# espnet/espnet

Hardware: AMD Instinct MI355X
Metric: audio-seconds/sec (RTF^-1), Conformer-ASR, 10 s utterances (higher is better)
Workload: dtype bf16; 1 GPU; BASELINE.json configs[1]: Conformer-small (12x256d, 4 heads), HIP STFT/log-mel + HIP encoder + greedy CTC (G1) + hypotheses collated to the host, 32 x 10 s utterances per GPU per step, V=5000; batch_per_gpu=32, global_batch=32, parallelism=utterance-dp1

## Files before the change

### espnet_amd/asr/encoder/conformer_encoder.py

```python
import ctypes as C
import math
import os
import threading
import weakref
from typing import List, Optional, Tuple

import torch

from espnet_amd import lib as L
from espnet_amd.nets_utils import (SUBSAMPLING_CONVS, SUBSAMPLING_MIN_FRAMES, conv2d_subsampled_lengths,
                                   conv_out_size)
from espnet_amd.packing import PackedModule

_POS_PROJ_LOCK = threading.Lock()
_ENC_CALL_LOCK = threading.Lock()
_TLS = threading.local()

LN_EPS = 1e-12


class LayerNorm(torch.nn.LayerNorm):
    def __init__(self, nout):
        super().__init__(nout, eps=LN_EPS)


class _Conv2dSubsampling(torch.nn.Module):

# ... 410 lines not shown
    def _pack_current(self, pk) -> bool:
        stamp = getattr(pk, "ctc_stamp", None)
        return stamp is None or self.fused_ctc is None or stamp == self._ctc_version(self.fused_ctc)

    def _pack_subsampling(self, w, t, A, F):
        e, d = self.embed, self._output_size
        layer = getattr(self, "input_layer", "conv2d")
        w.subsample = {"conv2d": 4, "conv2d6": 6, "conv2d8": 8}[layer]
        w.legacy_relpos = int(getattr(self, "legacy_relpos", False))
        k2 = e.conv[2].weight.size(-1)
        t["conv2_w"] = A(e.conv[2].weight.permute(0, 2, 3, 1).reshape(d, k2 * k2 * d))
        t["conv2_b"] = F(e.conv[2].bias)
        if layer == "conv2d" and d in (256, 512) and self.em_dtype == L.EM_BF16:
            t["conv1_wf"] = A(pack_conv1_frags(e.conv[0].weight, e.conv[0].bias))
            t["conv2_wf"] = A(pack_conv2_frags(e.conv[2].weight.permute(0, 2, 3, 1).reshape(d, 9 * d)))
        if layer == "conv2d8":
            t["conv3_w"] = A(e.conv[4].weight.permute(0, 2, 3, 1).reshape(d, 9 * d))
            t["conv3_b"] = F(e.conv[4].bias)

    def _pos_projected(self, T: int, device, pk, pos: torch.Tensor) -> torch.Tensor:
        cache = self.__dict__.setdefault("_pos_proj_cache", {})
        lock = _POS_PROJ_LOCK
        key = (T, str(device), pk.serial)
        cur = torch.cuda.current_stream()
        with lock:
            ent = cache.get(key)
            if ent is not None:
                out, ev, sid, _ = ent
                if sid != cur.cuda_stream:
                    cur.wait_event(ev)
# ... 151 lines not shown
```

### espnet_amd/csrc/api.hip

```cpp
#include <stdlib.h>

#include <atomic>
#include <mutex>

#include "em_common.h"
#include "switches.h"

namespace {
EmSwitches read_switches() {
  auto on = [](const char* n) { return getenv(n) != nullptr; };
  auto num = [](const char* n, int dflt) { const char* e = getenv(n); return e ? atoi(e) : dflt; };
  EmSwitches s = {};
  s.attn2_stamps = on("EM_ATTN2_STAMPS"); s.block_stamps = on("EM_BLOCK_STAMPS"); s.ffn_stamps = on("EM_FFN_STAMPS");
  s.sub2_stamps = on("EM_SUB2_STAMPS");
  s.block_no_helpers = on("ESPNET_AMD_BLOCK_NO_HELPERS");
  s.sa_split = num("ESPNET_AMD_SA_SPLIT", 0); s.sa_group = num("ESPNET_AMD_SA_GROUP", 0);
  s.no_sa_tree = on("ESPNET_AMD_NO_SA_TREE"); s.sa_tree_min_rows = num("ESPNET_AMD_SA_TREE_MIN_ROWS", 200);
  s.no_attn2_large = on("ESPNET_AMD_NO_ATTN2_LARGE"); s.no_ffn_rows = on("ESPNET_AMD_NO_FFN_ROWS");
  s.no_rows_ctc = on("ESPNET_AMD_NO_ROWS_CTC"); s.frontend_v1 = on("ESPNET_AMD_FRONTEND_V1");
  s.gemm_stages = num("ESPNET_AMD_GEMM_STAGES", 0); s.gemm_bm = num("ESPNET_AMD_GEMM_BM", 0); s.no_mid_gemm = on("ESPNET_AMD_NO_MID_GEMM");
  s.mid_tile = num("ESPNET_AMD_MID_TILE", 0); s.lng_rt = num("ESPNET_AMD_LNG_RT", 0); s.lng_wide = num("ESPNET_AMD_LNG_WIDE", 256);
  s.no_src_lnq = on("ESPNET_AMD_NO_SRC_LNQ"); s.no_tail_fusion = on("ESPNET_AMD_NO_TAIL_FUSION");
  s.stream_no_fused = on("ESPNET_AMD_STREAM_NO_FUSED"); s.stream_mha_v1 = on("ESPNET_AMD_STREAM_MHA_V1");
  s.stream_no_ctx_fold = on("ESPNET_AMD_STREAM_NO_CTX_FOLD"); s.stream_no_ln_gemm = on("ESPNET_AMD_STREAM_NO_LN_GEMM");
  s.stream_fused_min = num("ESPNET_AMD_STREAM_FUSED_MIN", 1); s.no_sub12 = on("ESPNET_AMD_NO_SUB12");
  s.stream_ffn_split = num("ESPNET_AMD_STREAM_FFN_SPLIT", 0); s.stream_split_att = on("ESPNET_AMD_STREAM_SPLIT_ATT");
  s.stream_tf_merge = num("ESPNET_AMD_STREAM_TF_MERGE", -1);
  s.dec_ffn_split = num("ESPNET_AMD_DEC_FFN_SPLIT", 0); s.dec_ffn_rows = num("ESPNET_AMD_DEC_FFN_ROWS", 0); s.no_rows_qkv = on("ESPNET_AMD_NO_ROWS_QKV"); s.ffn_rows_min_fill = num("ESPNET_AMD_FFN_ROWS_MIN_FILL", 0);
  return s;
}
std::atomic<const EmSwitches*> g_sw{nullptr};
std::mutex g_sw_mu;
}

const EmSwitches& em_sw() {
  const EmSwitches* p = g_sw.load(std::memory_order_acquire);
  if (!p) {
    std::lock_guard<std::mutex> lk(g_sw_mu);
    p = g_sw.load(std::memory_order_acquire);
    if (!p) {
// ... 50 lines not shown
```

### espnet_amd/csrc/ebranchformer.hip

```cpp
#include <math.h>
#include <stdlib.h>

#include "em_common.h"
#include "switches.h"
#include "subsample.h"

namespace {

constexpr float LN_EPS = 1e-12f;

inline size_t align_up(size_t v) { return (v + 255) & ~(size_t)255; }

struct Ws {
  size_t c1, c2, c3, x, xn, xn2, big, gn, gated, cat, tmp, ctx, pall, mw, qh, kh, vt, total;
  int Tpad;
};
inline Ws layout(int dtype, const EmEBranchformerWeights* w, int B, int T_f) {
  const size_t es = dtype == EM_BF16 ? 2 : 4;
  em_sub::Geo g;
  em_sub::geo(w->subsample, T_f, w->n_mels, &g);
  const size_t M = (size_t)B * g.T_out, d = w->d;
  size_t mb[3];
  em_sub::map_bytes(g, B, w->d, es, mb);
  size_t wide = w->ff > 3 * w->d ? w->ff : 3 * w->d;
// ... 155 lines not shown
  void* c1 = ws + s.c1;
  void* c2 = ws + s.c2;
  void* c3 = ws + s.c3;
  float* x = (float*)(ws + s.x);
  void* xn = ws + s.xn;
  void* xn2 = ws + s.xn2;
  void* big = ws + s.big;
  void* gn = ws + s.gn;
  void* gated = ws + s.gated;
  unsigned char* cat = ws + s.cat;
  void* tmp = ws + s.tmp;
  void* ctx = ws + s.ctx;
  void* pall = ws + s.pall;
  const size_t es = dtype == EM_BF16 ? 2 : 4;

  EM_TRY(em_sub::run(dtype, w, g, feats, mvn_partial, flens, B, c1, c2, c3, x, stream, w->conv1_wf, w->conv2_wf));
  EM_TRY(gemm(dtype, EM_EPI_STORE, pos_emb, w->wpos_all, pall, nullptr, w->legacy_relpos ? T : 2 * T - 1, L * d, d, d, L * d, 1.f,
              stream));
  const EmEBranchformerLayer* ly = w->layers;
  const bool ffn = w->use_ffn != 0;
  const bool no_attn2 = em_sw().no_attn2_large;
  const bool attn2 = dtype == EM_BF16 && !w->legacy_relpos && !no_attn2 && !(flags & EM_ENC_NO_FUSED) && d == 64 * h &&
                     (size_t)B * d * s.Tpad * 4 < ((size_t)1 << 32) - 64;
  void* qh = ws + s.qh;
  void* vt = ws + s.vt;
  if (attn2 && hipMemsetAsync(qh, 0, (s.vt - s.qh) + (size_t)B * d * s.Tpad * es, (hipStream_t)stream) != hipSuccess)
    return EM_ERR_LAUNCH;
  bool ffn_rows = ffn && dtype == EM_BF16 && d == 512 && ff % 128 == 0 && ff >= 256 && !(flags & EM_ENC_NO_FUSED) &&
                  !em_sw().no_ffn_rows && em_rows_fill_ok(M, flags);
  for (int l = 0; ffn_rows && l < L; ++l) ffn_rows = ly[l].ffm_w1p && ly[l].ffm_w2p && ly[l].ff_w1p && ly[l].ff_w2p;
  const EmEBranchformerLayer* ln_in = nullptr;
// ... 105 lines not shown
```

### espnet_amd/csrc/em_common.h

```cpp
#pragma once
#include <hip/hip_runtime.h>
#include <stdint.h>

#include <mutex>

#include "../../include/espnet_amd.h"

typedef __bf16 bf16;
typedef __attribute__((ext_vector_type(8))) __bf16 bf16x8;
typedef __attribute__((ext_vector_type(4))) __bf16 bf16x4;
typedef __attribute__((ext_vector_type(2))) __bf16 bf16x2;
typedef __attribute__((ext_vector_type(4))) float f32x4;
typedef __attribute__((ext_vector_type(2))) float f32x2;

#define EM_WAVE 64

template <typename T>
struct Mma;

template <>
struct Mma<bf16> {
  static constexpr int K = 32;
  static constexpr int EPL = 8;
  typedef bf16x8 frag;
// ... 124 lines not shown
  int dev = 0;
  if (hipGetDevice(&dev) != hipSuccess || dev < 0 || dev >= 64) return EM_ERR_LAUNCH;
  if ((int)bytes > __atomic_load_n(&cap->bytes[dev], __ATOMIC_ACQUIRE)) {
    std::lock_guard<std::mutex> lk(em_lds_cap_mu);
    if ((int)bytes > __atomic_load_n(&cap->bytes[dev], __ATOMIC_RELAXED)) {
      if (hipFuncSetAttribute(fn, hipFuncAttributeMaxDynamicSharedMemorySize, (int)bytes) != hipSuccess) return EM_ERR_LAUNCH;
      __atomic_store_n(&cap->bytes[dev], (int)bytes, __ATOMIC_RELEASE);
    }
  }
  return EM_OK;
}

bool em_prof_begin(void* stream);
void em_prof_end(void* stream, double flops, int tag);

bool em_rows_fill_ok(long M, int flags);

int em_dec_pack_memory_frag_bf16(const void* kv, int B, int T, int Tpad, int d, int heads, void* kf, void* vf, void* stream);
int em_dec_src_attention_lnq_memfrag_bf16(const float* x, const float* g, const float* be, float eps, const void* wq_frag,
                                          const float* bq, const void* kf, const void* vf, const int32_t* klens, int B, int W, int d,
                                          int heads, int T, int Tpad, void* ctx, void* stream);

int em_gemm_mid_frag(int epilogue, int frag, const EmGemmArgs* p, void* stream);

int em_dec_self_attention_tree_bf16(const void* qkv, void* kc, void* vc, const int* anc, const int* anc_odd, int n, int d,
                                    int heads, int Lmax, int pos, const int* pos_dev, int W, void* ctx, void* stream);

struct NgSearchArgs {
  int32_t n, W, V, Lmax, S, NC;
  float w_ctc, w_ngram;
  const int32_t* step;
// ... 10 lines not shown
```

### espnet_amd/csrc/encoder.hip

```cpp
#include <math.h>
#include <stdlib.h>

#include "em_common.h"
#include "switches.h"
#include "subsample.h"

namespace {

constexpr float LN_EPS = 1e-12f;

inline size_t align_up(size_t v) { return (v + 255) & ~(size_t)255; }

struct Ws {
  size_t c1, c2, c3, x, xn, big, g, g2, ctx, pall, qh, kh, vt, ppk, total;
  int Tpad;
};
inline int fused_tpad(int T) { return (T + 255) / 256 * 256; }
inline Ws layout(int dtype, const EmConformerWeights* w, int B, int T_f) {
  const size_t es = dtype == EM_BF16 ? 2 : 4;
  em_sub::Geo g;
  em_sub::geo(w->subsample, T_f, w->n_mels, &g);
  const size_t M = (size_t)B * g.T_out, d = w->d;
  size_t mb[3];
  em_sub::map_bytes(g, B, w->d, es, mb);
// ... 20 lines not shown
  return s;
}

inline int gemm(int dtype, int epi, const void* A, const void* W, void* C, const float* bias, int M,
                int N, int K, int lda, int ldc, float scale, void* stream) {
  EmGemmArgs a = {};
  a.A = A; a.W = W; a.C = C; a.bias = bias;
  a.M = M; a.N = N; a.K = K; a.lda = lda; a.ldc = ldc; a.scale = scale;
  a.T1 = a.F1 = a.T2 = a.F2 = a.d = 0;
  return em_gemm(dtype, epi, EM_A_PLAIN, &a, stream);
}


}

bool em_rows_fill_ok(long M, int flags) {
  static int n_cu_of[64] = {};
  int dev = 0;
  if (hipGetDevice(&dev) != hipSuccess || dev < 0 || dev >= 64) dev = 0;
  if (n_cu_of[dev] == 0) {
    hipDeviceProp_t prop;
    n_cu_of[dev] = (hipGetDeviceProperties(&prop, dev) == hipSuccess && prop.multiProcessorCount > 0) ? prop.multiProcessorCount : 256;
  }
  const int n_cu = n_cu_of[dev];
  int n = (flags >> 8) & 15;
  n = n < 1 ? 1 : n;
  const int forced = em_sw().ffn_rows_min_fill;
  const long fill = forced > 0 ? forced : 72 / n;
  const long wgs = (M + 63) / 64, rounds = (wgs + n_cu - 1) / n_cu;
  return M > 0 && 100 * wgs >= fill * rounds * n_cu;
}

namespace {

struct RowsPlan {
  bool ffn, pre_pw2, glu, ctc;
};
inline RowsPlan rows_plan(int dtype, const EmConformerWeights* w, int flags, long M) {
  RowsPlan r = {false, false, false, false};
  const bool no_ffn_rows = em_sw().no_ffn_rows;
  const int d = w->d, ff = w->ff, L = w->num_blocks;
  const EmConformerLayer* ly = w->layers;
  if (!(dtype == EM_BF16 && d == 512 && ff % 128 == 0 && ff >= 256 && !(flags & EM_ENC_NO_FUSED) && !no_ffn_rows && ly && L > 0 &&
        M > 0))
// ... 68 lines not shown
  if (!em_sub::geo(w->subsample, T_f, w->n_mels, &g)) return EM_ERR_UNSUPPORTED;
  const int T = g.T_out, M = B * T;
  unsigned char* ws = (unsigned char*)workspace;
  void* c1 = ws + s.c1;
  void* c2 = ws + s.c2;
  void* c3 = ws + s.c3;
  float* x = (float*)(ws + s.x);
  void* xn = ws + s.xn;
  void* big = ws + s.big;
  void* gl = ws + s.g;
  void* g2 = ws + s.g2;
  void* ctx = ws + s.ctx;
  void* pall = ws + s.pall;
  const size_t es = dtype == EM_BF16 ? 2 : 4;

  EM_TRY(em_sub::run(dtype, w, g, feats, mvn_partial, flens, B, c1, c2, c3, x, stream, w->conv1_wf, w->conv2_wf));
  const EmConformerLayer* ly = w->layers;
  if (flags & EM_ENC_POS_PROJECTED)
    pall = const_cast<void*>(pos_emb);
  else
    EM_TRY(gemm(dtype, EM_EPI_STORE, pos_emb, w->wpos_all, pall, nullptr, w->legacy_relpos ? T : 2 * T - 1, L * d, d, d,
                L * d, 1.f, stream));
  const int plan = encode_plan(dtype, w, flags);
  const bool fused = (plan & EM_ENC_PLAN_FUSED) != 0;
  if (fused) {
    void* qh = ws + s.qh;
    void* kh = ws + s.kh;
    void* vt = ws + s.vt;
    if (32 * em_cdiv(T, 32) < s.Tpad &&
        hipMemsetAsync(vt, 0, (size_t)B * d * s.Tpad * es, (hipStream_t)stream) != hipSuccess)
      return EM_ERR_LAUNCH;
// ... 176 lines not shown
```

### espnet_amd/csrc/subsample.h

```cpp
#pragma once
#include "switches.h"
#include <math.h>
#include <stdlib.h>

#include "em_common.h"

namespace em_sub {

struct Geo {
  int n;
  int T[4], F[4];
  int k[3], s[3];
  int T_out, F_out;
};

inline int mode_of(int subsample) { return subsample == 0 ? 4 : subsample; }

inline int min_frames(int subsample) {
  switch (mode_of(subsample)) {
    case 6: return 11;
    case 8: return 15;
    default: return 7;
  }
}
// ... 12 lines not shown
    g->F[i + 1] = (g->F[i] - g->k[i]) / g->s[i] + 1;
    if (g->T[i] < g->k[i] || g->F[i] < g->k[i]) return false;
  }
  g->T_out = g->T[convs];
  g->F_out = g->F[convs];
  return g->T_out >= 1 && g->F_out >= 1;
}

inline void map_bytes(const Geo& g, int B, int d, size_t es, size_t out[3]) {
  for (int i = 0; i < 3; ++i) out[i] = i <= g.n ? (size_t)B * g.T[i + 1] * g.F[i + 1] * d * es : 0;
}

template <typename W>
inline int run(int dtype, const W* w, const Geo& g, const float* feats, const float* mvn_partial,
               const int32_t* flens, int B, void* c1, void* c2, void* c3, float* x, void* stream,
               const void* conv1_wf = nullptr, const void* conv2_wf = nullptr) {
  const int d = w->d;
  int rc = EM_ERR_UNSUPPORTED;
  const bool no_fused = em_sw().no_sub12;
  const bool try_fused = dtype == EM_BF16 && conv1_wf && conv2_wf && mode_of(w->subsample) == 4 && !no_fused;
  if (try_fused)
    rc = em_conv2d_sub12_bf16(feats, mvn_partial, flens, B, g.T[0], g.F[0], conv1_wf, conv2_wf, w->conv2_b, d, c2, stream);
  if (rc != EM_OK && rc != EM_ERR_UNSUPPORTED) return rc;
  const bool fused = rc == EM_OK;
  if (!fused) {
    rc = em_conv2d_sub1(dtype, feats, mvn_partial, flens, B, g.T[0], g.F[0], w->conv1_w, w->conv1_b, d, c1, stream);
    if (rc != EM_OK) return rc;
  }
  const void* in = fused ? c2 : c1;
  void* outs[2] = {c2, c3};
  const void* ws[2] = {w->conv2_w, w->conv3_w};
  const float* bs[2] = {w->conv2_b, w->conv3_b};
  for (int i = fused ? 1 : 0; i < g.n; ++i) {
    EmGemmArgs a = {};
    a.A = in; a.W = ws[i]; a.C = outs[i]; a.bias = bs[i];
    a.M = B * g.T[i + 2] * g.F[i + 2]; a.N = d; a.K = g.k[i + 1] * g.k[i + 1] * d; a.lda = 0; a.ldc = d; a.scale = 1.f;
    a.T1 = g.T[i + 1]; a.F1 = g.F[i + 1]; a.T2 = g.T[i + 2]; a.F2 = g.F[i + 2]; a.d = d;
    a.conv_k = g.k[i + 1]; a.conv_s = g.s[i + 1];
    if (!a.W || !a.C) return EM_ERR_BAD_ARG;
    rc = em_gemm(dtype, EM_EPI_RELU, EM_A_CONV2, &a, stream);
    if (rc != EM_OK) return rc;
    in = outs[i];
  }
  EmGemmArgs e = {};
  e.A = in; e.W = w->embed_w; e.C = x; e.bias = w->embed_b;
  e.M = B * g.T_out; e.N = d; e.K = g.F_out * d; e.lda = g.F_out * d; e.ldc = d; e.scale = sqrtf((float)d);
  return em_gemm(dtype, EM_EPI_SCALE_F32, EM_A_PLAIN, &e, stream);
}

}
```

### espnet_amd/csrc/switches.h

```cpp
#pragma once

struct EmSwitches {
  bool attn2_stamps, block_stamps, ffn_stamps, sub2_stamps;
  bool block_no_helpers;
  int sa_split, sa_group;
  bool no_sa_tree;
  int sa_tree_min_rows;
  bool no_rows_qkv;
  bool no_attn2_large, no_ffn_rows, no_rows_ctc;
  bool frontend_v1;
  int gemm_stages, gemm_bm;
  bool no_mid_gemm;
  int mid_tile, lng_rt, lng_wide;
  bool no_src_lnq, no_tail_fusion;
  bool stream_no_fused, stream_mha_v1, stream_no_ctx_fold, stream_no_ln_gemm;
  int stream_fused_min;
  bool stream_split_att;
  int stream_ffn_split;
  int stream_tf_merge;
  bool no_sub12;
  int ffn_rows_min_fill;
  int dec_ffn_rows;
  int dec_ffn_split;
};

const EmSwitches& em_sw();
```

### espnet_amd/csrc/transformer.hip

```cpp
#include <math.h>
#include <stdlib.h>

#include "em_common.h"
#include "switches.h"
#include "subsample.h"

namespace {

constexpr float LN_EPS = 1e-12f;

inline size_t align_up(size_t v) { return (v + 255) & ~(size_t)255; }

struct Ws {
  size_t c1, c2, c3, x, xn, big, ctx, qh, kh, vt, total;
  int Tpad;
};
inline Ws layout(int dtype, const EmTransformerWeights* w, int B, int T_f) {
  const size_t es = dtype == EM_BF16 ? 2 : 4;
  em_sub::Geo g;
  em_sub::geo(w->subsample, T_f, w->n_mels, &g);
  const size_t M = (size_t)B * g.T_out, d = w->d;
  size_t mb[3];
  em_sub::map_bytes(g, B, w->d, es, mb);
  const size_t wide = (size_t)w->ff > 3 * d ? (size_t)w->ff : 3 * d;
// ... 64 lines not shown
  em_sub::Geo g;
  if (!em_sub::geo(w->subsample, T_f, w->n_mels, &g)) return EM_ERR_UNSUPPORTED;
  const int T = g.T_out, M = B * T;
  const size_t es = dtype == EM_BF16 ? 2 : 4;
  unsigned char* ws = (unsigned char*)workspace;
  float* x = (float*)(ws + s.x);
  void* xn = ws + s.xn;
  void* big = ws + s.big;
  void* ctx = ws + s.ctx;
  void* qh = ws + s.qh;
  void* kh = ws + s.kh;
  void* vt = ws + s.vt;
  hipStream_t hs = (hipStream_t)stream;

  EM_TRY(em_sub::run(dtype, w, g, feats, mvn_partial, flens, B, ws + s.c1, ws + s.c2, ws + s.c3, x, stream, w->conv1_wf,
                     w->conv2_wf));
  {
    const long n4 = (long)M * d / 4;
    hipLaunchKernelGGL(abs_pe_add_kernel, dim3((unsigned)((n4 + 255) / 256)), dim3(256), 0, hs, x, (const float*)pos_emb, T,
                       d / 4, n4);
    EM_CHECK_LAUNCH();
  }
  const EmTransformerLayer* ly = w->layers;
  if (L == 0)
    return em_layernorm(dtype, x, w->after_norm_g, w->after_norm_b, M, d, LN_EPS, enc_act, enc_out, stream);

  const bool heads_path = dtype == EM_BF16 && !em_sw().no_attn2_large && (size_t)B * d * s.Tpad * 4 < ((size_t)1 << 32) - 64;
  bool ffn_rows = dtype == EM_BF16 && d == 512 && ff % 128 == 0 && ff >= 256 && !(flags & EM_ENC_NO_FUSED) &&
                  !em_sw().no_ffn_rows && em_rows_fill_ok(M, flags);
  for (int l = 0; ffn_rows && l < L; ++l) ffn_rows = ly[l].ff_w1p && ly[l].ff_w2p;

// ... 43 lines not shown
```

### espnet_amd/lib.py

```python
import ctypes as C
import os
from pathlib import Path

_LIB_PATH = Path(__file__).resolve().parent / "lib" / "libespnet_amd.so"

EM_OK = 0
EM_LNF_RELU_FRAG, EM_LNF_STORE, EM_LNF_STORE_F32 = 0, 1, 2
EM_ERR_UNSUPPORTED, EM_ERR_BAD_ARG, EM_ERR_TOO_SHORT, EM_ERR_LAUNCH, EM_ERR_WORKSPACE, EM_ERR_IO = -1, -2, -3, -4, -5, -6
EM_F32, EM_BF16 = 0, 1
(EM_EPI_STORE, EM_EPI_SWISH, EM_EPI_RELU, EM_EPI_RESID_F32, EM_EPI_SCALE_F32, EM_EPI_GLU,
 EM_EPI_STORE_F32, _EM_EPI_UNUSED_7, _EM_EPI_UNUSED_8, EM_EPI_ARGMAX_PART, EM_EPI_GELU, EM_EPI_QK_HEADS,
 EM_EPI_VT_HEADS) = range(13)
EM_A_PLAIN, EM_A_CONV2 = 0, 1

EM_DW_SWISH, EM_DW_LINEAR, EM_DW_GATE, EM_DW_SELFRES = range(4)
EM_ENC_ISOLATE_UTTS = 1
EM_ENC_NO_FUSED = 2
EM_ENC_POS_PROJECTED = 4
EM_ENC_FOLD_C = 8
EM_ENC_SPLIT_ATT = 16
EM_ENC_POS_PACKED = 32


def EM_ENC_IN_FLIGHT(n):
# ... 64 lines not shown
               [(n, C.c_void_p) for n in ("pre_in", "pre_w", "pre_b", "pre_g", "pre_be")] + [("main", C.c_int32)] + \
               [(n, C.c_void_p) for n in ("post_w", "post_b", "post_ids")] + [("post_chunks", C.c_int32), ("post_vocab", C.c_int32)] + \
               [(n, C.c_void_p) for n in ("post_q", "post_k", "post_vt")] + [("post_T", C.c_int32), ("post_Tpad", C.c_int32)] + \
               [("act", C.c_int32)]


class EmConformerWeights(C.Structure):
    _fields_ = [("d", C.c_int32), ("heads", C.c_int32), ("ff", C.c_int32),
                ("num_blocks", C.c_int32), ("kernel", C.c_int32), ("n_mels", C.c_int32),
                ("conv1_w", C.c_void_p), ("conv1_b", C.c_void_p), ("conv2_w", C.c_void_p),
                ("conv2_b", C.c_void_p), ("embed_w", C.c_void_p), ("embed_b", C.c_void_p),
                ("wpos_all", C.c_void_p), ("after_norm_g", C.c_void_p),
                ("after_norm_b", C.c_void_p), ("layers", C.POINTER(EmConformerLayer)),
                ("subsample", C.c_int32), ("conv3_w", C.c_void_p), ("conv3_b", C.c_void_p),
                ("legacy_relpos", C.c_int32), ("ctc_w", C.c_void_p), ("ctc_b", C.c_void_p),
                ("ctc_ids", C.c_void_p), ("ctc_units", C.c_int32), ("conv1_wf", C.c_void_p), ("conv2_wf", C.c_void_p)]


_EBF_LAYER_PTRS = ["norm_ff_mac_g", "norm_ff_mac_b", "norm_mha_g", "norm_mha_b", "norm_mlp_g", "norm_mlp_b",
                   "norm_ff_g", "norm_ff_b", "norm_final_g", "norm_final_b", "ffm_w1", "ffm_w2", "ff_w1", "ff_w2",
                   "ffm_b1", "ffm_b2", "ff_b1", "ff_b2", "wqkv", "bqkv", "pos_u", "pos_v", "wout", "bout",
                   "proj1_w", "proj1_b", "csgu_norm_g", "csgu_norm_b", "csgu_conv_w", "csgu_conv_b", "proj2_w",
                   "proj2_b", "merge_conv_w", "merge_conv_b", "merge_w", "merge_b", "pool_w", "pool_b", "wproj_w",
                   "wproj_b", "ffm_w1p", "ffm_w2p", "ff_w1p", "ff_w2p", "wqkvp"]
EM_MERGE_CONCAT, EM_MERGE_LEARNED_AVE = 0, 1


class EmEBranchformerLayer(C.Structure):
    _fields_ = [(n, C.c_void_p) for n in _EBF_LAYER_PTRS]


class EmEBranchformerWeights(C.Structure):
    _fields_ = [(n, C.c_int32) for n in ("d", "heads", "ff", "cg", "num_blocks", "cg_kernel", "merge_kernel",
                                         "n_mels")] + \
               [(n, C.c_void_p) for n in ("conv1_w", "conv1_b", "conv2_w", "conv2_b", "embed_w", "embed_b",
                                          "wpos_all", "after_norm_g", "after_norm_b")] + \
               [("layers", C.POINTER(EmEBranchformerLayer)), ("use_ffn", C.c_int32), ("merge_conv", C.c_int32),
                ("subsample", C.c_int32), ("conv3_w", C.c_void_p), ("conv3_b", C.c_void_p),
                ("legacy_relpos", C.c_int32), ("merge_method", C.c_int32), ("conv1_wf", C.c_void_p),
                ("conv2_wf", C.c_void_p)]


_TRF_LAYER_PTRS = ["norm1_g", "norm1_b", "norm2_g", "norm2_b", "wqkv", "bqkv", "wout", "bout", "ff_w1", "ff_w2", "ff_b1",
                   "ff_b2", "ff_w1p", "ff_w2p", "cb_wqkvp", "cb_woutp", "cb_ff_w1p", "cb_ff_w2p", "fp_t"]


class EmTransformerLayer(C.Structure):
    _fields_ = [(n, C.c_void_p) for n in _TRF_LAYER_PTRS]


class EmTransformerWeights(C.Structure):
    _fields_ = [(n, C.c_int32) for n in ("d", "heads", "ff", "num_blocks", "n_mels", "subsample")] + \
               [(n, C.c_void_p) for n in ("conv1_w", "conv1_b", "conv2_w", "conv2_b", "conv3_w", "conv3_b", "embed_w",
                                          "embed_b", "after_norm_g", "after_norm_b")] + \
               [("layers", C.POINTER(EmTransformerLayer)), ("conv1_wf", C.c_void_p), ("conv2_wf", C.c_void_p)]


class EmWavInfo(C.Structure):
    _fields_ = [("frames", C.c_int64), ("data_offset", C.c_int64), ("rate", C.c_int32), ("channels", C.c_int32),
                ("bits", C.c_int32), ("format", C.c_int32), ("status", C.c_int32)]


_DEC_LAYER_PTRS = ["norm1_g", "norm1_b", "norm2_g", "norm2_b", "norm3_g", "norm3_b", "self_wqkv",
                   "self_bqkv", "self_wout", "self_bout", "src_wq", "src_bq", "src_wkv", "src_bkv",
                   "src_wout", "src_bout", "w1", "b1", "w2", "b2", "w1_frag", "w2_frag", "self_wqkv_frag",
                   "self_wout_frag", "src_wout_frag", "src_wq_frag"]


def pack_frag16(w, pad_rows=16):
    import torch
# ... 79 lines not shown
class EmSearchBuffers(C.Structure):
    _fields_ = [(n, C.c_void_p) for n in SEARCH_BUFFERS]


_i32, _f32, _vp, _sz = C.c_int32, C.c_float, C.c_void_p, C.c_size_t
_SIGNATURES = {
    "em_version": (C.c_int, []),
    "em_error_string": (C.c_char_p, [C.c_int]),
    "em_frontend_logmel_f32": (C.c_int, [_vp, _i32, _i32, _i32, _vp, _vp, _vp, _i32, _i32, _vp, _vp,
                                         _i32, _vp, _vp]),
    "em_utt_mvn_partial_f32": (C.c_int, [_vp, _vp, _i32, _i32, _i32, _vp, _vp]),
    "em_utt_mvn_apply_f32": (C.c_int, [_vp, _vp, _vp, _i32, _i32, _i32, _vp]),
    "em_global_mvn_f32": (C.c_int, [_vp, _vp, _vp, _vp, _i32, _i32, _i32, _vp]),
    "em_conv2d_sub1": (C.c_int, [C.c_int, _vp, _vp, _vp, _i32, _i32, _i32, _vp, _vp, _i32, _vp, _vp]),
    "em_conv2d_sub12_bf16": (C.c_int, [_vp, _vp, _vp, _i32, _i32, _i32, _vp, _vp, _vp, _i32, _vp, _vp]),
    "em_gemm": (C.c_int, [C.c_int, C.c_int, C.c_int, C.POINTER(EmGemmArgs), _vp]),
    "em_layernorm": (C.c_int, [C.c_int, _vp, _vp, _vp, _i32, _i32, _f32, _vp, _vp, _vp]),
    "em_layernorm2": (C.c_int, [C.c_int, _vp, _vp, _vp, _vp, _vp, _i32, _i32, _f32, _vp, _vp, _vp]),
    "em_layernorm_inplace_f32": (C.c_int, [_vp, _vp, _vp, _i32, _i32, _f32, _vp]),
    "em_relpos_attention": (C.c_int, [C.c_int, _vp, _vp, _i32, _vp, _vp, _vp, _i32, _i32, _i32,
                                      _i32, _vp, _vp]),
    "em_legacy_relpos_attention": (C.c_int, [C.c_int, _vp, _vp, _i32, _vp, _vp, _vp, _i32, _i32, _i32,
                                      _i32, _vp, _vp]),
    "em_dwconv_bn_swish": (C.c_int, [C.c_int, _vp, _vp, _vp, _vp, _i32, _i32, _i32, _i32, _vp, _vp]),
    "em_argmax_rows_f32": (C.c_int, [_vp, _i32, _i32, _vp, _vp]),
    "em_argmax_partials": (C.c_int, [_vp, _i32, _i32, _vp, _vp]),
    "em_log_softmax_rows_f32": (C.c_int, [_vp, _i32, _i32, _vp]),
    "em_ctc_collapse": (C.c_int, [_vp, _vp, _i32, _i32, _i32, _i32, _vp, _vp, _vp]),
    "em_conformer_workspace_bytes": (_sz, [C.c_int, C.POINTER(EmConformerWeights), _i32, _i32]),
    "em_ebranchformer_workspace_bytes": (_sz, [C.c_int, C.POINTER(EmEBranchformerWeights), _i32, _i32]),
# ... 156 lines not shown
```

### espnet_amd/packing.py

```python
import itertools
import threading

import torch

from espnet_amd import lib as L

_BUILD_LOCK = threading.RLock()
_SERIALS = itertools.count(1)


class Pack:

    def __init__(self, device: torch.device, dtype, act: torch.dtype, pe_len):
        self.device, self.dtype, self.act, self.pe_len = device, dtype, act, pe_len
        self.serial = next(_SERIALS)
        self.w = self.layers = None
        self.keep = []
        self._held = set()
        self._frozen = False

    def __setattr__(self, name, value):
        if self.__dict__.get("_frozen"):
            raise AttributeError(f"a pack does not change once built ({name})")
        object.__setattr__(self, name, value)
# ... 64 lines not shown
```

### include/espnet_amd.h

```cpp
#ifndef ESPNET_AMD_H_
#define ESPNET_AMD_H_

#include <stddef.h>
#include <stdint.h>

#ifdef __cplusplus
extern "C" {
#endif

#define EM_OK 0
#define EM_ERR_UNSUPPORTED (-1)
#define EM_ERR_BAD_ARG (-2)
#define EM_ERR_TOO_SHORT (-3)
#define EM_ERR_LAUNCH (-4)
#define EM_ERR_WORKSPACE (-5)
#define EM_ERR_IO (-6)

#define EM_F32 0
#define EM_BF16 1

#define EM_EPI_STORE 0
#define EM_EPI_SWISH 1
#define EM_EPI_RELU 2
#define EM_EPI_RESID_F32 3
// ... 33 lines not shown
                           int32_t n_mels, float* partial, void* stream);

int em_utt_mvn_apply_f32(float* feats, const float* partial, const int32_t* flens, int32_t B,
                         int32_t T_f, int32_t n_mels, void* stream);

int em_global_mvn_f32(float* feats, const int32_t* flens, const float* mean, const float* stdv,
                      int32_t B, int32_t T_f, int32_t n_mels, void* stream);

int em_conv2d_sub12_bf16(const float* feats, const float* mvn_partial, const int32_t* flens, int32_t B, int32_t T_f,
                         int32_t n_mels, const void* conv1_wf, const void* conv2_wf, const float* conv2_b, int32_t d,
                         void* c2, void* stream);

int em_conv2d_sub1(int dtype, const float* feats, const float* partial, const int32_t* flens,
                   int32_t B, int32_t T_f, int32_t n_mels, const float* w1, const float* b1,
                   int32_t d, void* out, void* stream);

int em_gemm(int dtype, int epilogue, int a_mode, const EmGemmArgs* args, void* stream);

int em_layernorm(int dtype, const float* x, const float* g, const float* b, int32_t M, int32_t d,
                 float eps, void* out, float* out_f32, void* stream);
int em_layernorm2(int dtype, float* x, const float* g1, const float* b1, const float* g2,
                  const float* b2, int32_t M, int32_t d, float eps, void* out, float* out_f32,
                  void* stream);

int em_layernorm_inplace_f32(float* x, const float* g, const float* b, int32_t M, int32_t d,
                             float eps, void* stream);

int em_ln_gemm(int dtype, int epilogue, const float* x, const float* ln_g, const float* ln_b, float eps,
               const void* W, const float* bias, void* C, int32_t M, int32_t N, int32_t K, int32_t ldc,
               void* stream);
// ... 70 lines not shown
  const void* embed_w;
  const float* embed_b;
  const void* wpos_all;
  const float *after_norm_g, *after_norm_b;
  const EmConformerLayer* layers;
  int32_t subsample;
  const void* conv3_w;
  const float* conv3_b;
  int32_t legacy_relpos;
  const void* ctc_w;
  const float* ctc_b;
  int32_t* ctc_ids;
  int32_t ctc_units;
  const void* conv1_wf;
  const void* conv2_wf;
} EmConformerWeights;

#define EM_ENC_ISOLATE_UTTS 1
#define EM_ENC_NO_FUSED 2
#define EM_ENC_FOLD_C 8
#define EM_ENC_SPLIT_ATT 16
#define EM_ENC_POS_PACKED 32
#define EM_ENC_POS_PROJECTED 4
#define EM_ENC_IN_FLIGHT(n) (((n) & 15) << 8)

#define EM_ENC_PLAN_FUSED 1
#define EM_ENC_PLAN_CTC_IDS 2
int em_conformer_encode_plan(int dtype, const EmConformerWeights* w, int32_t flags);
int em_conformer_encode_plan_for(int dtype, const EmConformerWeights* w, int32_t flags, int32_t B, int32_t T_f);

// ... 108 lines not shown

typedef struct EmTransformerWeights {
  int32_t d, heads, ff, num_blocks, n_mels;
  int32_t subsample;
  const float *conv1_w, *conv1_b;
  const void* conv2_w;
  const float* conv2_b;
  const void* conv3_w;
  const float* conv3_b;
  const void* embed_w;
  const float* embed_b;
  const float *after_norm_g, *after_norm_b;
  const EmTransformerLayer* layers;
  const void* conv1_wf;
  const void* conv2_wf;
} EmTransformerWeights;

size_t em_transformer_workspace_bytes(int dtype, const EmTransformerWeights* w, int32_t B, int32_t T_f);
int em_transformer_encode(int dtype, const EmTransformerWeights* w, const float* feats, const float* mvn_partial,
                          const int32_t* flens, const int32_t* olens, int32_t B, int32_t T_f, const void* pos_emb,
                          void* workspace, size_t workspace_bytes, float* enc_out, void* enc_act, int32_t flags,
                          void* stream);

typedef struct EmEBranchformerLayer {
  const float *norm_ff_mac_g, *norm_ff_mac_b, *norm_mha_g, *norm_mha_b, *norm_mlp_g, *norm_mlp_b;
  const float *norm_ff_g, *norm_ff_b, *norm_final_g, *norm_final_b;
  const void *ffm_w1, *ffm_w2, *ff_w1, *ff_w2;
  const float *ffm_b1, *ffm_b2, *ff_b1, *ff_b2;
  const void* wqkv;
  const float* bqkv;
// ... 25 lines not shown
  const float* conv2_b;
  const void* embed_w;
  const float* embed_b;
  const void* wpos_all;
  const float *after_norm_g, *after_norm_b;
  const EmEBranchformerLayer* layers;
  int32_t use_ffn;
  int32_t merge_conv;
  int32_t subsample;
  const void* conv3_w;
  const float* conv3_b;
  int32_t legacy_relpos;
  int32_t merge_method;
  const void* conv1_wf;
  const void* conv2_wf;
} EmEBranchformerWeights;

int em_branch_learned_ave(int dtype, const void* cat, const int32_t* lens, int32_t B, int32_t T, int32_t d,
                          const float* pool_w, const float* pool_b, const float* wproj_w,
                          const float* wproj_b, float* mw_ws, void* out, void* stream);

size_t em_ebranchformer_workspace_bytes(int dtype, const EmEBranchformerWeights* w, int32_t B, int32_t T_f);
int em_ebranchformer_encode(int dtype, const EmEBranchformerWeights* w, const float* feats,
                            const float* mvn_partial, const int32_t* flens, const int32_t* olens,
                            int32_t B, int32_t T_f, const void* pos_emb, void* workspace,
                            size_t workspace_bytes, float* enc_out, void* enc_act, int32_t flags,
                            void* stream);

int em_ctc_greedy(int dtype, const void* enc_act, const void* w_ctc, const float* b_ctc, int32_t B,
                  int32_t T, int32_t d, int32_t V, const int32_t* olens, int32_t blank,
// ... 300 lines not shown
```

Before: 354,700 audio-s/s.

## Add row-tiled MFMA kernel for subsampling embed projection with pre-packed weights

Adds a dedicated bf16 kernel for the Conv2dSubsampling output linear (embed) projection. It streams activation tiles into LDS with global_load_lds through a 4-stage ring and keeps pre-packed weight fragments in a register ring, fusing bias and sqrt(d) scaling into the store. Weights are repacked on the host at pack time into the fragment order. The kernel is used when the CU fill heuristic allows it, otherwise the generic GEMM runs. It aims to cut the generic GEMM's cost on this large-K, small-N shape, at the price of more code and a new packed-weight buffer.

```diff
diff --git a/espnet_amd/asr/encoder/conformer_encoder.py b/espnet_amd/asr/encoder/conformer_encoder.py
--- a/espnet_amd/asr/encoder/conformer_encoder.py
+++ b/espnet_amd/asr/encoder/conformer_encoder.py
@@ -10,7 +10,7 @@
 from espnet_amd import lib as L
 from espnet_amd.nets_utils import (SUBSAMPLING_CONVS, SUBSAMPLING_MIN_FRAMES, conv2d_subsampled_lengths,
                                    conv_out_size)
-from espnet_amd.packing import PackedModule
+from espnet_amd.packing import PackedModule, pack_embed_rows
 
 _POS_PROJ_LOCK = threading.Lock()
 _ENC_CALL_LOCK = threading.Lock()
@@ -451,6 +451,9 @@
         if layer == "conv2d" and d in (256, 512) and self.em_dtype == L.EM_BF16:
             t["conv1_wf"] = A(pack_conv1_frags(e.conv[0].weight, e.conv[0].bias))
             t["conv2_wf"] = A(pack_conv2_frags(e.conv[2].weight.permute(0, 2, 3, 1).reshape(d, 9 * d)))
+        F_out = e.out.in_features // d
+        if d in (256, 512) and self.em_dtype == L.EM_BF16 and (F_out * d) % 256 == 0:
+            t["embed_wf"] = A(pack_embed_rows(e.out.weight.reshape(d, d, F_out).permute(0, 2, 1).reshape(d, F_out * d)))
         if layer == "conv2d8":
             t["conv3_w"] = A(e.conv[4].weight.permute(0, 2, 3, 1).reshape(d, 9 * d))
             t["conv3_b"] = F(e.conv[4].bias)
diff --git a/espnet_amd/csrc/api.hip b/espnet_amd/csrc/api.hip
--- a/espnet_amd/csrc/api.hip
+++ b/espnet_amd/csrc/api.hip
@@ -24,6 +24,7 @@
   s.stream_no_fused = on("ESPNET_AMD_STREAM_NO_FUSED"); s.stream_mha_v1 = on("ESPNET_AMD_STREAM_MHA_V1");
   s.stream_no_ctx_fold = on("ESPNET_AMD_STREAM_NO_CTX_FOLD"); s.stream_no_ln_gemm = on("ESPNET_AMD_STREAM_NO_LN_GEMM");
   s.stream_fused_min = num("ESPNET_AMD_STREAM_FUSED_MIN", 1); s.no_sub12 = on("ESPNET_AMD_NO_SUB12");
+  s.no_embed_rows = on("ESPNET_AMD_NO_EMBED_ROWS");
   s.stream_ffn_split = num("ESPNET_AMD_STREAM_FFN_SPLIT", 0); s.stream_split_att = on("ESPNET_AMD_STREAM_SPLIT_ATT");
   s.stream_tf_merge = num("ESPNET_AMD_STREAM_TF_MERGE", -1);
   s.dec_ffn_split = num("ESPNET_AMD_DEC_FFN_SPLIT", 0); s.dec_ffn_rows = num("ESPNET_AMD_DEC_FFN_ROWS", 0); s.no_rows_qkv = on("ESPNET_AMD_NO_ROWS_QKV"); s.ffn_rows_min_fill = num("ESPNET_AMD_FFN_ROWS_MIN_FILL", 0);
diff --git a/espnet_amd/csrc/ebranchformer.hip b/espnet_amd/csrc/ebranchformer.hip
--- a/espnet_amd/csrc/ebranchformer.hip
+++ b/espnet_amd/csrc/ebranchformer.hip
@@ -193,7 +193,7 @@
   void* pall = ws + s.pall;
   const size_t es = dtype == EM_BF16 ? 2 : 4;
 
-  EM_TRY(em_sub::run(dtype, w, g, feats, mvn_partial, flens, B, c1, c2, c3, x, stream, w->conv1_wf, w->conv2_wf));
+  EM_TRY(em_sub::run(dtype, w, g, feats, mvn_partial, flens, B, c1, c2, c3, x, stream, w->conv1_wf, w->conv2_wf, w->embed_wf, flags));
   EM_TRY(gemm(dtype, EM_EPI_STORE, pos_emb, w->wpos_all, pall, nullptr, w->legacy_relpos ? T : 2 * T - 1, L * d, d, d, L * d, 1.f,
               stream));
   const EmEBranchformerLayer* ly = w->layers;
diff --git a/espnet_amd/csrc/em_common.h b/espnet_amd/csrc/em_common.h
--- a/espnet_amd/csrc/em_common.h
+++ b/espnet_amd/csrc/em_common.h
@@ -162,7 +162,7 @@
 bool em_prof_begin(void* stream);
 void em_prof_end(void* stream, double flops, int tag);
 
-bool em_rows_fill_ok(long M, int flags);
+bool em_rows_fill_ok(long M, int flags, int rows = 64);
 
 int em_dec_pack_memory_frag_bf16(const void* kv, int B, int T, int Tpad, int d, int heads, void* kf, void* vf, void* stream);
 int em_dec_src_attention_lnq_memfrag_bf16(const float* x, const float* g, const float* be, float eps, const void* wq_frag,
diff --git a/espnet_amd/csrc/embed_rows.hip b/espnet_amd/csrc/embed_rows.hip
--- /dev/null
+++ b/espnet_amd/csrc/embed_rows.hip
@@ -0,0 +1,175 @@
+#include <stdlib.h>
+
+#include "em_common.h"
+#include "switches.h"
+
+namespace {
+
+typedef const __attribute__((address_space(1))) unsigned char* GU8;
+typedef const __attribute__((address_space(1))) bf16x8* GFRAG;
+
+__device__ __forceinline__ void glds16(const unsigned char* sbase, unsigned voff, unsigned lds_dst) {
+  unsigned keep;
+  asm volatile(
+      "s_nop 4\n\t"
+      "s_mov_b32 %0, m0\n\t"
+      "s_mov_b32 m0, %3\n\t"
+      "s_nop 0\n\t"
+      "global_load_lds_dwordx4 %1, %2\n\t"
+      "s_mov_b32 m0, %0"
+      : "=&s"(keep)
+      : "v"(voff), "s"(sbase), "s"(lds_dst)
+      : "memory");
+}
+
+__device__ __forceinline__ const unsigned char* uniform_ptr(const unsigned char* p) {
+  const unsigned long long v = (unsigned long long)p;
+  const unsigned lo = __builtin_amdgcn_readfirstlane((unsigned)v);
+  const unsigned hi = __builtin_amdgcn_readfirstlane((unsigned)(v >> 32));
+  return (const unsigned char*)(((unsigned long long)hi << 32) | lo);
+}
+
+constexpr int NS = 4;
+constexpr int KT_STAGE = 4;
+constexpr int SU = 8;
+
+template <int D>
+struct Shape {
+  static constexpr int NCF = D / 64;
+  static constexpr int MI = D / 128;
+  static constexpr int ROWS = 16 * MI;
+  static constexpr int RING = 2048 / D;
+  static constexpr int KT_BYTES = ROWS * 128;
+  static constexpr int STAGE = KT_STAGE * KT_BYTES;
+  static constexpr int PIECES = ROWS / 32;
+  static constexpr int LDS = NS * STAGE;
+  static constexpr unsigned UNIT = D * 64;
+  static_assert(SU % RING == 0 && (NS - 2) * SU * NCF >= 63 && LDS <= 160 * 1024, "ring / stage shape");
+};
+
+template <int D>
+__global__ __launch_bounds__(256, 1) void embed_rows_kernel(const unsigned char* __restrict__ A, const unsigned char* __restrict__ Wf,
+                                                            const float* __restrict__ bias, float* __restrict__ X, int M, int K,
+                                                            unsigned lda_bytes, float scale) {
+  using S = Shape<D>;
+  using MM = Mma<bf16>;
+  constexpr int NCF = S::NCF, MI = S::MI, RING = S::RING;
+  extern __shared__ __attribute__((aligned(1024))) unsigned char smem[];
+  const unsigned lds0 = (unsigned)(size_t)(__attribute__((address_space(3))) unsigned char*)smem;
+
+  const int tid = threadIdx.x, lane = tid & 63;
+  const int wave = __builtin_amdgcn_readfirstlane(tid >> 6);
+  const int lr = lane & 15, lg = lane >> 4;
+  const int m0 = blockIdx.x * S::ROWS;
+  const int nst = K / (64 * KT_STAGE), nu = K / 32;
+
+  unsigned voff[S::PIECES];
+#pragma unroll
+  for (int p = 0; p < S::PIECES; ++p) {
+    int m = m0 + (wave + 4 * p) * 8 + (lane >> 3);
+    m = m < M ? m : M - 1;
+    voff[p] = (unsigned)m * lda_bytes + (((lane & 7) ^ (lane >> 3)) << 4);
+  }
+  auto dma = [&](int st, int slot) __attribute__((always_inline)) {
+    st = st < nst ? st : nst - 1;
+#pragma unroll
+    for (int j = 0; j < KT_STAGE; ++j) {
+      const unsigned char* src = uniform_ptr(A + (size_t)(st * KT_STAGE + j) * 128);
+#pragma unroll
+      for (int p = 0; p < S::PIECES; ++p)
+        glds16(src, voff[p], __builtin_amdgcn_readfirstlane(lds0 + slot * S::STAGE + j * S::KT_BYTES + (wave + 4 * p) * 1024));
+    }
+  };
+  bf16x8 ring[RING][NCF];
+  GU8 const wbase = (GU8)Wf + wave * (NCF * 1024) + lane * 16;
+  auto read_unit = [&](int u, bf16x8 (&w)[NCF]) __attribute__((always_inline)) {
+    u = u < nu ? u : nu - 1;
+    GU8 su = wbase + (size_t)u * S::UNIT;
+#pragma unroll
+    for (int cf = 0; cf < NCF; ++cf) w[cf] = *(GFRAG)(su + cf * 1024);
+  };
+
+  float4 b4[NCF];
+#pragma unroll
+  for (int cf = 0; cf < NCF; ++cf) b4[cf] = *(const float4*)(bias + (wave * NCF + cf) * 16 + lg * 4);
+#pragma unroll
+  for (int s = 0; s < NS - 1; ++s) dma(s, s);
+#pragma unroll
+  for (int u = 0; u < RING; ++u) read_unit(u, ring[u]);
+
+  f32x4 acc[MI][NCF];
+#pragma unroll
+  for (int mi = 0; mi < MI; ++mi)
+#pragma unroll
+    for (int cf = 0; cf < NCF; ++cf) acc[mi][cf] = (f32x4){0.f, 0.f, 0.f, 0.f};
+
+  asm volatile("s_waitcnt vmcnt(%0)" ::"n"(RING * NCF) : "memory");
+  __builtin_amdgcn_s_barrier();
+
+  const int frag_rd = lr * 128;
+  const int swz = lr & 7;
+#pragma unroll 1
+  for (int kt = 0; kt < nst; ++kt) {
+    dma(kt + NS - 1, (kt + NS - 1) & (NS - 1));
+    const unsigned char* sa = smem + (kt & (NS - 1)) * S::STAGE + frag_rd;
+#pragma unroll
+    for (int j = 0; j < SU; ++j) {
+      bf16x8 fb[MI];
+#pragma unroll
+      for (int mi = 0; mi < MI; ++mi)
+        fb[mi] = *(const bf16x8*)(sa + (j >> 1) * S::KT_BYTES + mi * 2048 + ((((j & 1) * 4 + lg) ^ swz) << 4));
+#pragma unroll
+      for (int cf = 0; cf < NCF; ++cf)
+#pragma unroll
+        for (int mi = 0; mi < MI; ++mi) acc[mi][cf] = MM::mma(ring[j % RING][cf], fb[mi], acc[mi][cf]);
+      read_unit(kt * SU + j + RING, ring[j % RING]);
+    }
+    asm volatile("s_waitcnt vmcnt(63) lgkmcnt(0)" ::: "memory");
+    __builtin_amdgcn_s_barrier();
+  }
+  asm volatile("s_waitcnt vmcnt(0)" ::: "memory");
+
+  const __amdgpu_buffer_rsrc_t rs = __builtin_amdgcn_make_buffer_rsrc(X, 0, (int)(unsigned)((size_t)M * D * 4), 0x00020000);
+#pragma unroll
+  for (int mi = 0; mi < MI; ++mi) {
+    const int m = m0 + mi * 16 + lr;
+#pragma unroll
+    for (int cf = 0; cf < NCF; ++cf) {
+      const f32x4 c = acc[mi][cf];
+      float4 v = make_float4(c[0] + b4[cf].x, c[1] + b4[cf].y, c[2] + b4[cf].z, c[3] + b4[cf].w);
+      v.x *= scale; v.y *= scale; v.z *= scale; v.w *= scale;
+      typedef __attribute__((ext_vector_type(4))) unsigned u32x4;
+      const u32x4 raw = {__float_as_uint(v.x), __float_as_uint(v.y), __float_as_uint(v.z), __float_as_uint(v.w)};
+      const unsigned off = m < M ? (unsigned)(((size_t)m * D + (wave * NCF + cf) * 16 + lg * 4) * 4) : 0xffffffffu;
+      __builtin_amdgcn_raw_buffer_store_b128(raw, rs, off, 0, 0);
+    }
+  }
+}
+
+template <int D>
+int launch(const void* c2, const void* wf, const float* bias, float* x, int M, int K, int lda, float scale, hipStream_t s) {
+  using S = Shape<D>;
+  auto* fn = embed_rows_kernel<D>;
+  static EmLdsCap cap = {};
+  if (S::LDS > 64 * 1024 && em_raise_lds_cap((const void*)fn, S::LDS, &cap) != EM_OK) return EM_ERR_LAUNCH;
+  hipLaunchKernelGGL(fn, dim3(em_cdiv(M, S::ROWS)), dim3(256), S::LDS, s, (const unsigned char*)c2, (const unsigned char*)wf, bias, x, M,
+                     K, (unsigned)lda * 2u, scale);
+  EM_CHECK_LAUNCH();
+  return EM_OK;
+}
+
+}
+
+extern "C" int em_embed_rows_bf16(const void* c2, const void* w_frag, const float* bias, float* x, int32_t M, int32_t d, int32_t K,
+                                  int32_t lda, float scale, void* stream) {
+  if (!c2 || !w_frag || !bias || !x || M <= 0 || K <= 0) return EM_ERR_BAD_ARG;
+  if (d != 256 && d != 512) return EM_ERR_UNSUPPORTED;
+  if (K % (64 * KT_STAGE) != 0 || lda < K || lda % 8 != 0) return EM_ERR_UNSUPPORTED;
+  if ((size_t)M * lda * 2 >= ((size_t)1 << 32) || (size_t)M * d * 4 >= ((size_t)1 << 32) - 64) return EM_ERR_UNSUPPORTED;
+  if (((size_t)c2 | (size_t)w_frag | (size_t)bias | (size_t)x) & 15) return EM_ERR_UNSUPPORTED;
+  const bool rec = em_prof_begin(stream);
+  const int rc = d == 256 ? launch<256>(c2, w_frag, bias, x, M, K, lda, scale, (hipStream_t)stream)
+                          : launch<512>(c2, w_frag, bias, x, M, K, lda, scale, (hipStream_t)stream);
+  if (rec) em_prof_end(stream, 2.0 * (double)M * (double)d * (double)K, EM_PROF_GEMM);
+  return rc;
+}
diff --git a/espnet_amd/csrc/encoder.hip b/espnet_amd/csrc/encoder.hip
--- a/espnet_amd/csrc/encoder.hip
+++ b/espnet_amd/csrc/encoder.hip
@@ -58,7 +58,7 @@
 
 }
 
-bool em_rows_fill_ok(long M, int flags) {
+bool em_rows_fill_ok(long M, int flags, int rows) {
   static int n_cu_of[64] = {};
   int dev = 0;
   if (hipGetDevice(&dev) != hipSuccess || dev < 0 || dev >= 64) dev = 0;
@@ -71,7 +71,7 @@
   n = n < 1 ? 1 : n;
   const int forced = em_sw().ffn_rows_min_fill;
   const long fill = forced > 0 ? forced : 72 / n;
-  const long wgs = (M + 63) / 64, rounds = (wgs + n_cu - 1) / n_cu;
+  const long wgs = (M + rows - 1) / rows, rounds = (wgs + n_cu - 1) / n_cu;
   return M > 0 && 100 * wgs >= fill * rounds * n_cu;
 }
 
@@ -170,7 +170,7 @@
   void* pall = ws + s.pall;
   const size_t es = dtype == EM_BF16 ? 2 : 4;
 
-  EM_TRY(em_sub::run(dtype, w, g, feats, mvn_partial, flens, B, c1, c2, c3, x, stream, w->conv1_wf, w->conv2_wf));
+  EM_TRY(em_sub::run(dtype, w, g, feats, mvn_partial, flens, B, c1, c2, c3, x, stream, w->conv1_wf, w->conv2_wf, w->embed_wf, flags));
   const EmConformerLayer* ly = w->layers;
   if (flags & EM_ENC_POS_PROJECTED)
     pall = const_cast<void*>(pos_emb);
diff --git a/espnet_amd/csrc/subsample.h b/espnet_amd/csrc/subsample.h
--- a/espnet_amd/csrc/subsample.h
+++ b/espnet_amd/csrc/subsample.h
@@ -50,7 +50,7 @@
 template <typename W>
 inline int run(int dtype, const W* w, const Geo& g, const float* feats, const float* mvn_partial,
                const int32_t* flens, int B, void* c1, void* c2, void* c3, float* x, void* stream,
-               const void* conv1_wf = nullptr, const void* conv2_wf = nullptr) {
+               const void* conv1_wf = nullptr, const void* conv2_wf = nullptr, const void* embed_wf = nullptr, int flags = 0) {
   const int d = w->d;
   int rc = EM_ERR_UNSUPPORTED;
   const bool no_fused = em_sw().no_sub12;
@@ -81,6 +81,10 @@
   EmGemmArgs e = {};
   e.A = in; e.W = w->embed_w; e.C = x; e.bias = w->embed_b;
   e.M = B * g.T_out; e.N = d; e.K = g.F_out * d; e.lda = g.F_out * d; e.ldc = d; e.scale = sqrtf((float)d);
+  if (dtype == EM_BF16 && embed_wf && (d == 256 || d == 512) && !em_sw().no_embed_rows && em_rows_fill_ok(e.M, flags, d / 8)) {
+    rc = em_embed_rows_bf16(e.A, embed_wf, w->embed_b, x, e.M, d, e.K, e.lda, e.scale, stream);
+    if (rc != EM_ERR_UNSUPPORTED) return rc;
+  }
   return em_gemm(dtype, EM_EPI_SCALE_F32, EM_A_PLAIN, &e, stream);
 }
 
diff --git a/espnet_amd/csrc/switches.h b/espnet_amd/csrc/switches.h
--- a/espnet_amd/csrc/switches.h
+++ b/espnet_amd/csrc/switches.h
@@ -19,6 +19,7 @@
   int stream_ffn_split;
   int stream_tf_merge;
   bool no_sub12;
+  bool no_embed_rows;
   int ffn_rows_min_fill;
   int dec_ffn_rows;
   int dec_ffn_split;
diff --git a/espnet_amd/csrc/transformer.hip b/espnet_amd/csrc/transformer.hip
--- a/espnet_amd/csrc/transformer.hip
+++ b/espnet_amd/csrc/transformer.hip
@@ -102,7 +102,7 @@
   hipStream_t hs = (hipStream_t)stream;
 
   EM_TRY(em_sub::run(dtype, w, g, feats, mvn_partial, flens, B, ws + s.c1, ws + s.c2, ws + s.c3, x, stream, w->conv1_wf,
-                     w->conv2_wf));
+                     w->conv2_wf, w->embed_wf, flags));
   {
     const long n4 = (long)M * d / 4;
     hipLaunchKernelGGL(abs_pe_add_kernel, dim3((unsigned)((n4 + 255) / 256)), dim3(256), 0, hs, x, (const float*)pos_emb, T,
diff --git a/espnet_amd/lib.py b/espnet_amd/lib.py
--- a/espnet_amd/lib.py
+++ b/espnet_amd/lib.py
@@ -102,7 +102,8 @@
                 ("after_norm_b", C.c_void_p), ("layers", C.POINTER(EmConformerLayer)),
                 ("subsample", C.c_int32), ("conv3_w", C.c_void_p), ("conv3_b", C.c_void_p),
                 ("legacy_relpos", C.c_int32), ("ctc_w", C.c_void_p), ("ctc_b", C.c_void_p),
-                ("ctc_ids", C.c_void_p), ("ctc_units", C.c_int32), ("conv1_wf", C.c_void_p), ("conv2_wf", C.c_void_p)]
+                ("ctc_ids", C.c_void_p), ("ctc_units", C.c_int32), ("conv1_wf", C.c_void_p), ("conv2_wf", C.c_void_p),
+                ("embed_wf", C.c_void_p)]
 
 
 _EBF_LAYER_PTRS = ["norm_ff_mac_g", "norm_ff_mac_b", "norm_mha_g", "norm_mha_b", "norm_mlp_g", "norm_mlp_b",
@@ -126,7 +127,7 @@
                [("layers", C.POINTER(EmEBranchformerLayer)), ("use_ffn", C.c_int32), ("merge_conv", C.c_int32),
                 ("subsample", C.c_int32), ("conv3_w", C.c_void_p), ("conv3_b", C.c_void_p),
                 ("legacy_relpos", C.c_int32), ("merge_method", C.c_int32), ("conv1_wf", C.c_void_p),
-                ("conv2_wf", C.c_void_p)]
+                ("conv2_wf", C.c_void_p), ("embed_wf", C.c_void_p)]
 
 
 _TRF_LAYER_PTRS = ["norm1_g", "norm1_b", "norm2_g", "norm2_b", "wqkv", "bqkv", "wout", "bout", "ff_w1", "ff_w2", "ff_b1",
@@ -141,7 +142,8 @@
     _fields_ = [(n, C.c_int32) for n in ("d", "heads", "ff", "num_blocks", "n_mels", "subsample")] + \
                [(n, C.c_void_p) for n in ("conv1_w", "conv1_b", "conv2_w", "conv2_b", "conv3_w", "conv3_b", "embed_w",
                                           "embed_b", "after_norm_g", "after_norm_b")] + \
-               [("layers", C.POINTER(EmTransformerLayer)), ("conv1_wf", C.c_void_p), ("conv2_wf", C.c_void_p)]
+               [("layers", C.POINTER(EmTransformerLayer)), ("conv1_wf", C.c_void_p), ("conv2_wf", C.c_void_p),
+                ("embed_wf", C.c_void_p)]
 
 
 class EmWavInfo(C.Structure):
@@ -251,6 +253,7 @@
     "em_global_mvn_f32": (C.c_int, [_vp, _vp, _vp, _vp, _i32, _i32, _i32, _vp]),
     "em_conv2d_sub1": (C.c_int, [C.c_int, _vp, _vp, _vp, _i32, _i32, _i32, _vp, _vp, _i32, _vp, _vp]),
     "em_conv2d_sub12_bf16": (C.c_int, [_vp, _vp, _vp, _i32, _i32, _i32, _vp, _vp, _vp, _i32, _vp, _vp]),
+    "em_embed_rows_bf16": (C.c_int, [_vp, _vp, _vp, _vp, _i32, _i32, _i32, _i32, _f32, _vp]),
     "em_gemm": (C.c_int, [C.c_int, C.c_int, C.c_int, C.POINTER(EmGemmArgs), _vp]),
     "em_layernorm": (C.c_int, [C.c_int, _vp, _vp, _vp, _i32, _i32, _f32, _vp, _vp, _vp]),
     "em_layernorm2": (C.c_int, [C.c_int, _vp, _vp, _vp, _vp, _vp, _i32, _i32, _f32, _vp, _vp, _vp]),
diff --git a/espnet_amd/packing.py b/espnet_amd/packing.py
--- a/espnet_amd/packing.py
+++ b/espnet_amd/packing.py
@@ -4,6 +4,13 @@
 import torch
 
 from espnet_amd import lib as L
+
+def pack_embed_rows(w: torch.Tensor) -> torch.Tensor:
+    d, k = w.shape
+    assert d in (256, 512) and k % 32 == 0, (d, k)
+    u = w.detach().reshape(4, d // 64, 16, k // 32, 4, 8).permute(3, 0, 1, 4, 2, 5).contiguous()
+    return u.reshape(d, k)
+
 
 _BUILD_LOCK = threading.RLock()
 _SERIALS = itertools.count(1)
diff --git a/include/espnet_amd.h b/include/espnet_amd.h
--- a/include/espnet_amd.h
+++ b/include/espnet_amd.h
@@ -71,6 +71,9 @@
 int em_conv2d_sub1(int dtype, const float* feats, const float* partial, const int32_t* flens,
                    int32_t B, int32_t T_f, int32_t n_mels, const float* w1, const float* b1,
                    int32_t d, void* out, void* stream);
+
+int em_embed_rows_bf16(const void* c2, const void* w_frag, const float* bias, float* x, int32_t M, int32_t d, int32_t K,
+                       int32_t lda, float scale, void* stream);
 
 int em_gemm(int dtype, int epilogue, int a_mode, const EmGemmArgs* args, void* stream);
 
@@ -171,6 +174,7 @@
   int32_t ctc_units;
   const void* conv1_wf;
   const void* conv2_wf;
+  const void* embed_wf;
 } EmConformerWeights;
 
 #define EM_ENC_ISOLATE_UTTS 1
@@ -309,6 +313,7 @@
   const EmTransformerLayer* layers;
   const void* conv1_wf;
   const void* conv2_wf;
+  const void* embed_wf;
 } EmTransformerWeights;
 
 size_t em_transformer_workspace_bytes(int dtype, const EmTransformerWeights* w, int32_t B, int32_t T_f);
@@ -364,6 +369,7 @@
   int32_t merge_method;
   const void* conv1_wf;
   const void* conv2_wf;
+  const void* embed_wf;
 } EmEBranchformerWeights;
 
 int em_branch_learned_ave(int dtype, const void* cat, const int32_t* lens, int32_t B, int32_t T, int32_t d,
```

Result: no change. 352,900 audio-s/s (-0.5%).
